# ALVI-Labs/frankenstein

Hardware: AMD Instinct MI355X
Metric: neural frames/sec (train fwd+bwd+AdamW, whole job) (higher is better)
Workload: dtype bf16; 1 GPU; brainformer-small (6L d=384 6x64 heads, N=6144 tokens) + 2-block perceiver, L1 head; fwd+bwd+clip+AdamW; per_gpu_batch=32, global_batch=32, frames_T=600, electrodes=256, parallelism=dp1, weights=random-init (seed 42)

## Files before the change

frankenstein_amd/_lib.py:

```python
from __future__ import annotations

import ctypes as C
from pathlib import Path

import os

LIB_PATH = Path(os.environ.get("FRANKEN_HIP_LIB") or Path(__file__).resolve().parent / "libfranken_hip.so")

FK_F32, FK_BF16 = 0, 1
MASK_NONE, MASK_CAUSAL, MASK_BLOCK_CAUSAL, MASK_PREFIX, MASK_KEYPAD, MASK_DENSE = 0, 1, 2, 3, 4, 5
NORM_LAYER, NORM_RMS = 0, 1
ATTN_Q_PRESCALED = 1
GEMV_GELU = 1
NT_RING2, NT_RING192, NT_RING128, NT_BIG, NT_GLDS4, NT_GLDS, NT_STAGED = range(7)
NT_ROUTE_F32 = -2

_p, _i64, _int, _f32, _f64, _sz, _u32 = C.c_void_p, C.c_int64, C.c_int, C.c_float, C.c_double, C.c_size_t, C.c_uint32

SIGNATURES = {
    "fk_version": (_int, []),
    "fk_last_error": (C.c_char_p, []),
    "fk_gemm_nt": (_int, [_p, _i64, _p, _i64, _p, _i64, _i64, _i64, _i64, _p, _p, _i64, _i64, _int, _int, _p]),
    "fk_gemv_nt": (_int, [_p, _i64, _p, _i64, _p, _i64, _i64, _i64, _i64, _p, _p, _i64, _p, _p, _f32, _int, _int, _int, _p]),
    "fk_gemm_nt_rope": (_int, [_p, _i64, _p, _i64, _p, _i64, _i64, _i64, _i64, _p, _p, _i64, _i64, _i64, _i64, _i64, _i64, _i64, _int, _p]),
    "fk_gemm_nt_swiglu": (_int, [_p, _i64, _p, _i64, _p, _i64, _p, _i64, _i64, _i64, _i64, _int, _p]),
    "fk_gemm_nt_dswiglu": (_int, [_p, _i64, _p, _i64, _p, _i64, _p, _i64, _i64, _i64, _i64, _int, _p]),
    "fk_mlp_bwd_fused": (_int, [_p, _i64, _p, _i64, _p, _i64, _p, _i64, _p, _i64, _p, _i64, _i64, _i64, _i64, _int, _p]),
    "fk_gemm_nt_route": (_int, [_i64, _i64, _i64, _int, _int, _int, _int]),
    "fk_gemm_tn_route": (_int, [_i64, _i64, _i64, _int, _p, _p]),
    "fk_gemm_tn_workspace_bytes": (_sz, [_i64, _i64, _i64, _int]),
    "fk_gemm_tn": (_int, [_p, _i64, _p, _i64, _p, _i64, _i64, _i64, _i64, _int, _int, _p, _sz, _p]),
    "fk_colsum_workspace_bytes": (_sz, [_i64, _i64]),
    "fk_colsum": (_int, [_p, _i64, _p, _i64, _i64, _int, _int, _p, _sz, _p]),
    "fk_attn_fwd": (_int, [_p, _p, _p, _p, _p] + [_i64] * 13 + [_int, _i64, _i64, _i64, _p, _p, _f32, _int, _int, _p]),
    "fk_attn_bwd": (_int, [_p] * 10 + [_i64] * 13 + [_int, _i64, _i64, _i64, _p, _p, _f32, _p, _i64, _i64, _int, _int, _p]),
    "fk_attn_fwd_dropout": (_int, [_p, _p, _p, _p, _p] + [_i64] * 13 + [_int, _i64, _i64, _i64, _p, _p, _f32, _int, _f32, _p, _u32, _int, _p]),
    "fk_attn_bwd_dropout": (_int, [_p] * 10 + [_i64] * 13 + [_int, _i64, _i64, _i64, _p, _p, _f32, _p, _i64, _i64, _int, _f32, _p, _u32, _int, _p]),
    "fk_dropout": (_int, [_p, _p, _p, _i64, _f32, _p, _u32, _int, _p]),
    "fk_norm_fwd": (_int, [_p, _p, _p, _p, _p, _p, _i64, _i64, _f32, _int, _int, _p]),
    "fk_norm_bwd_workspace_bytes": (_sz, [_i64, _i64]),
    "fk_norm_bwd": (_int, [_p] * 9 + [_i64, _i64, _int, _int, _int, _p, _sz, _p]),
    "fk_rope": (_int, [_p, _i64, _i64, _i64, _i64, _i64, _p, _i64, _i64, _int, _int, _p]),
    "fk_patchify": (_int, [_p, _p, _i64, _i64, _i64, _i64, _i64, _int, _p]),
    "fk_swiglu_fwd": (_int, [_p, _p, _i64, _i64, _int, _p]),
    "fk_swiglu_bwd": (_int, [_p, _p, _p, _i64, _i64, _int, _p]),
    "fk_gelu_fwd": (_int, [_p, _p, _i64, _int, _p]),
    "fk_gelu_bwd": (_int, [_p, _p, _p, _i64, _int, _p]),
    "fk_cast_pack": (_int, [_p, _i64, _p, _i64, _i64, _i64, _int, _int, _p]),
    "fk_cast_pack_rows": (_int, [_p, _i64, _p, _i64, _i64, _i64, _int, _i64, _i64, _i64, _int, _p]),
    "fk_cast_pack_multi": (_int, [_p, _i64, _i64, _int, _p]),
    "fk_cast": (_int, [_p, _int, _p, _int, _i64, _p]),
    "fk_add": (_int, [_p, _p, _p, _i64, _int, _p]),
    "fk_gather_rows": (_int, [_p, _i64, _int, _p, _i64, _p, _i64, _int, _i64, _i64, _i64, _int, _p]),
    "fk_scatter_add_rows": (_int, [_p, _int, _p, _i64, _p, _i64, _i64, _p]),
    "fk_prefix_mask": (_int, [_p, _p, _i64, _p, _p, _i64, _i64, _i64, _p]),
    "fk_copy2d": (_int, [_p, _i64, _p, _i64, _i64, _i64, _int, _p]),
    "fk_attn_combine": (_int, [_p, _p, _p, _p, _i64, _i64, _i64, _i64, _i64, _int, _p]),
    "fk_add2d": (_int, [_p, _i64, _p, _i64, _i64, _i64, _p]),
    "fk_gpt_embed_step": (_int, [_p, _p, _p, _p, _p, _i64, _i64, _i64, _int, _p]),
    "fk_kv_append": (_int, [_p, _p, _p, _i64, _i64, _i64, _int, _p]),
    "fk_attn_decode": (_int, [_p, _i64, _p, _i64, _i64, _p, _i64, _p, _i64, _i64, _i64, _f32, _int, _p]),
    "fk_sample_topk": (_int, [_p, _i64, _i64, _i64, _f32, _i64, _p, _p, _p, _p, _p, _i64, _i64, _p, _p]),
    "fk_attn_decode_beam": (_int, [_p, _i64, _p, _i64, _i64, _p, _i64, _p, _i64, _p, _i64, _i64, _i64, _f32, _int, _p]),
    "fk_beam_topk": (_int, [_p, _i64, _i64, _i64, _f32, _i64, _p, _p, _p]),
# ... 64 lines not shown
```

frankenstein_amd/csrc/gemm.hip:

```cpp
#include <type_traits>

#include "fk_common.h"

namespace {

#ifndef FK_EPI_UNROLL
#define FK_EPI_UNROLL 1
#endif
#include "gemm_tile.h"

struct NtArgs {
  const void* A; const void* B; void* C;
  const void* bias; const void* res;
  int64_t lda, ldb, ldc, ldr, res_rows;
  int M, N, K, vec_epi;
  int mode;
  void* aux; int64_t ldaux;
  const float* rope_table; int64_t rope_bs; int rope_T, rope_off, rope_D, rope_cols;
  int rope_qcols; int64_t rope_qoff;
};

#ifndef FK_NT_STORES_GEMM
#define FK_NT_STORES_GEMM 1
#endif
// ... 1054 lines not shown
#pragma unroll
      for (int i = 0; i < 2; ++i) tn_frag<T>(fa[i], as, wm * 64 + i * 32, s, lane);
#pragma unroll
      for (int j = 0; j < 2; ++j) tn_frag<T>(fb[j], bs, wn * 64 + j * 32, s, lane);
#pragma unroll
      for (int i = 0; i < 2; ++i)
#pragma unroll
        for (int j = 0; j < 2; ++j) mma32<T>(acc[i][j], fa[i], fb[j]);
    }
    if (kt + 1 < nk) lstore((kt + 1) & 1);
    __syncthreads();
  }

  float* out = (p.nsplit > 1) ? p.ws + (int64_t)split * p.N1 * p.N2 : p.C;
  const int64_t ldo = (p.nsplit > 1) ? p.N2 : p.ldc;
  const bool accum = (p.nsplit == 1) && p.accumulate;
#pragma unroll
  for (int j = 0; j < 2; ++j) {
    const int n = b0 + wn * 64 + j * 32 + li;
    if (n >= p.N2) continue;
#pragma unroll
    for (int i = 0; i < 2; ++i)
#pragma unroll
      for (int r = 0; r < 16; ++r) {
        const int m = a0 + wm * 64 + i * 32 + acc_row(r, lh);
        if (m >= p.N1) continue;
        float* dst = out + (int64_t)m * ldo + n;
        *dst = accum ? (*dst + acc[i][j][r]) : acc[i][j][r];
      }
  }
}

constexpr int TG_A = 384, TG_B = 128, TG_K = 32;
#ifndef FK_TG_NS
#define FK_TG_NS 4
#endif
constexpr int TG_NS = FK_TG_NS;
constexpr int TG_A_ROW = TG_A * 2, TG_B_ROW = TG_B * 2;
constexpr int TG_A_BYTES = TG_K * TG_A_ROW, TG_B_BYTES = TG_K * TG_B_ROW, TG_STAGE = TG_A_BYTES + TG_B_BYTES;

template <int PITCH> FK_DEV int tg_off(int row, int bytecol) {
  return row * PITCH + (bytecol & ~255) + ((((bytecol >> 6) ^ row) & 3) << 6) + (bytecol & 63);
}
template <int OFF> FK_DEV bf16x4 tr_read(unsigned base) {
  s16x4 r;
  asm volatile("ds_read_b64_tr_b16 %0, %1 offset:%2" : "=v"(r) : "v"(base), "n"(OFF) : "memory");
  return __builtin_bit_cast(bf16x4, r);
}
template <int N> FK_DEV void lgkm_wait() {
  asm volatile("s_waitcnt lgkmcnt(%0)" ::"n"(N) : "memory");
  __builtin_amdgcn_sched_barrier(0);
}
template <int PITCH, int S> FK_DEV void tg_frag(Frag<bf16_t>& f, unsigned base) {
  const bf16x4 v0 = tr_read<(16 * S) * PITCH>(base), v1 = tr_read<(16 * S + 4) * PITCH>(base);
#pragma unroll
  for (int e = 0; e < 4; ++e) { f.v[e] = v0[e]; f.v[4 + e] = v1[e]; }
}
FK_DEV unsigned lds_addr(const char* p) {
  return (unsigned)(__UINTPTR_TYPE__)((__attribute__((address_space(3))) const char*)p);
}

template <int TB>
__global__ __launch_bounds__(512, 2) void gemm_tn_big_kernel(TnArgs p) {
  constexpr int B_ROW = TB == 128 ? 256 : 512, B_BYTES = TG_K * B_ROW, STAGE = TG_A_BYTES + B_BYTES, NJ = TB / 64, WB = TB / 2;
  using T = bf16_t;
  extern __shared__ __attribute__((aligned(16))) char smem[];
  const int tid = threadIdx.x, lane = tid & 63;
  const int wave = __builtin_amdgcn_readfirstlane(tid >> 6);
  const int wm = wave >> 1, wn = wave & 1, li = lane & 31, lh = lane >> 5;
  const int nt2 = p.N2 / TB, ntiles = (p.N1 / TG_A) * nt2;
  const unsigned L = xcd_remap(blockIdx.x, gridDim.x);
  const int split = (int)(L / ntiles), tile = (int)(L % ntiles);
  const int a0 = (tile / nt2) * TG_A, b0 = (tile % nt2) * TB;
  const int mbeg = split * p.rows_per_split;
  const int mend = min(p.M, mbeg + p.rows_per_split);
  const int nk = (mend - mbeg) / TG_K;

  constexpr int APW = TG_A_BYTES / 8192, BPW = B_BYTES / 8192, PER = APW + BPW;
  const T* srcA[APW];
  const T* srcB[BPW];
#pragma unroll
  for (int j = 0; j < APW; ++j) {
    const int o = (wave * APW + j) * 1024 + lane * 16, row = o / TG_A_ROW, bc = o % TG_A_ROW;
    const int sc = (bc & ~255) + ((((bc >> 6) ^ row) & 3) << 6) + (bc & 63);
    srcA[j] = (const T*)p.A + (int64_t)(mbeg + row) * p.lda + a0 + sc / 2;
  }
#pragma unroll
  for (int j = 0; j < BPW; ++j) {
    const int o = (wave * BPW + j) * 1024 + lane * 16, row = o / B_ROW, bc = o % B_ROW;
    int sc = (bc & ~255) + ((((bc >> 6) ^ row) & 3) << 6) + (bc & 63);
    if (sc >= TB * 2) sc = 0;
    srcB[j] = (const T*)p.B + (int64_t)(mbeg + row) * p.ldb + b0 + sc / 2;
  }
  const int64_t astep = (int64_t)TG_K * p.lda, bstep = (int64_t)TG_K * p.ldb;
  auto stage = [&](int buf) {
    char* as = smem + buf * STAGE;
#pragma unroll
    for (int j = 0; j < APW; ++j) {
      __builtin_amdgcn_global_load_lds((glb_void_t*)srcA[j], (lds_void_t*)(as + (wave * APW + j) * 1024), 16, 0, 0);
      srcA[j] += astep;
    }
#pragma unroll
    for (int j = 0; j < BPW; ++j) {
      __builtin_amdgcn_global_load_lds((glb_void_t*)srcB[j], (lds_void_t*)(as + TG_A_BYTES + (wave * BPW + j) * 1024), 16, 0, 0);
      srcB[j] += bstep;
    }
  };

  unsigned fbase[3 + NJ];
  {
    const int g = lane >> 4, i = lane & 15, row = 8 * (g >> 1) + (i >> 2), dc = 16 * (g & 1) + 4 * (i & 3);
#pragma unroll
    for (int q = 0; q < 3; ++q) fbase[q] = lds_addr(smem) + tg_off<TG_A_ROW>(row, (wm * 96 + q * 32 + dc) * 2);
#pragma unroll
    for (int q = 0; q < NJ; ++q) fbase[3 + q] = lds_addr(smem) + TG_A_BYTES + tg_off<B_ROW>(row, (wn * WB + q * 32 + dc) * 2);
  }

  f32x16 acc[3][NJ];
#pragma unroll
  for (int i = 0; i < 3; ++i)
#pragma unroll
    for (int j = 0; j < NJ; ++j)
#pragma unroll
      for (int r = 0; r < 16; ++r) acc[i][j][r] = 0.0f;

#pragma unroll
  for (int s = 0; s < TG_NS - 1; ++s)
    if (s < nk) stage(s);
  int slot = 0;
  for (int kt = 0; kt < nk; ++kt) {
    const int after = nk - 1 - kt;
    if (after >= TG_NS - 2) vm_wait_barrier<(TG_NS - 2) * PER>();
    else if (after == 3) vm_wait_barrier<3 * PER>();
    else if (after == 2) vm_wait_barrier<2 * PER>();
    else if (after == 1) vm_wait_barrier<PER>();
    else vm_wait_barrier<0>();
    if (kt + TG_NS - 1 < nk) stage(slot == 0 ? TG_NS - 1 : slot - 1);
    const unsigned bo = slot * STAGE;
    slot = slot == TG_NS - 1 ? 0 : slot + 1;
    Frag<T> f0[3 + NJ], f1[3 + NJ];
#pragma unroll
    for (int q = 0; q < 3; ++q) tg_frag<TG_A_ROW, 0>(f0[q], fbase[q] + bo);
#pragma unroll
    for (int q = 0; q < NJ; ++q) tg_frag<B_ROW, 0>(f0[3 + q], fbase[3 + q] + bo);
#pragma unroll
    for (int q = 0; q < 3; ++q) tg_frag<TG_A_ROW, 1>(f1[q], fbase[q] + bo);
#pragma unroll
    for (int q = 0; q < NJ; ++q) tg_frag<B_ROW, 1>(f1[3 + q], fbase[3 + q] + bo);
    lgkm_wait<2 * (3 + NJ)>();
#pragma unroll
    for (int i = 0; i < 3; ++i)
#pragma unroll
      for (int j = 0; j < NJ; ++j) mma32<T>(acc[i][j], f0[i], f0[3 + j]);
    lgkm_wait<0>();
#pragma unroll
    for (int i = 0; i < 3; ++i)
#pragma unroll
      for (int j = 0; j < NJ; ++j) mma32<T>(acc[i][j], f1[i], f1[3 + j]);
  }

  float* out = (p.nsplit > 1) ? p.ws + (int64_t)split * p.N1 * p.N2 : p.C;
  const int64_t ldo = (p.nsplit > 1) ? p.N2 : p.ldc;
  const bool accum = (p.nsplit == 1) && p.accumulate;
#pragma unroll
  for (int j = 0; j < NJ; ++j) {
    const int n = b0 + wn * WB + j * 32 + li;
#pragma unroll
    for (int i = 0; i < 3; ++i)
#pragma unroll
      for (int r = 0; r < 16; ++r) {
        const int m = a0 + wm * 96 + i * 32 + acc_row(r, lh);
        float* dst = out + (int64_t)m * ldo + n;
        *dst = accum ? (*dst + acc[i][j][r]) : acc[i][j][r];
      }
  }
}

__global__ __launch_bounds__(256) void reduce_slabs4_kernel(const float* ws, float* C, int64_t ldc, int N1, int N2, int nsplit, int accumulate) {
  const int64_t total = (int64_t)N1 * N2, total4 = total >> 2;
  const int n2v = N2 >> 2;
  for (int64_t i = blockIdx.x * (int64_t)blockDim.x + threadIdx.x; i < total4; i += (int64_t)gridDim.x * blockDim.x) {
    const f32x4* src = reinterpret_cast<const f32x4*>(ws) + i;
    f32x4 s = {0.0f, 0.0f, 0.0f, 0.0f};
    int k = 0;
    for (; k + 8 <= nsplit; k += 8) {
      f32x4 v[8];
#pragma unroll
      for (int u = 0; u < 8; ++u) v[u] = src[(int64_t)(k + u) * total4];
#pragma unroll
      for (int u = 0; u < 8; ++u) s += v[u];
    }
    for (; k < nsplit; ++k) s += src[(int64_t)k * total4];
    f32x4* dst = reinterpret_cast<f32x4*>(C + (i / n2v) * ldc + (i % n2v) * 4);
    if (accumulate) s += *dst;
    *dst = s;
  }
}
__global__ void reduce_slabs_kernel(const float* ws, float* C, int64_t ldc, int N1, int N2, int nsplit, int accumulate) {
  const int64_t total = (int64_t)N1 * N2;
  for (int64_t i = blockIdx.x * (int64_t)blockDim.x + threadIdx.x; i < total; i += (int64_t)gridDim.x * blockDim.x) {
    float s = 0.0f;
    for (int k = 0; k < nsplit; ++k) s += ws[k * total + i];
    float* dst = C + (i / N2) * ldc + (i % N2);
    *dst = accumulate ? (*dst + s) : s;
  }
}

template <typename T>
__global__ __launch_bounds__(256) void colsum_partial_kernel(const T* X, int64_t ld, float* part, int rows, int cols, int rows_per_blk) {
  constexpr int N = 16 / sizeof(T);
  __shared__ float red[256 * N];
  const int r0 = blockIdx.y * rows_per_blk, r1 = min(rows, r0 + rows_per_blk);
  const int cvt = (cols + N - 1) / N;
  {
    const int cv0 = blockIdx.x * 256;
    const int cvn = min(256, cvt - cv0), groups = 256 / cvn;
    const int vec = threadIdx.x % cvn, grp = threadIdx.x / cvn;
    float acc[N];
#pragma unroll
    for (int e = 0; e < N; ++e) acc[e] = 0.0f;
    if (grp < groups) {
      const T* p = X + (int64_t)(cv0 + vec) * N;
      for (int r = r0 + grp; r < r1; r += groups) {
        if constexpr (sizeof(T) == 2) {
          bf16x8 v = *reinterpret_cast<const bf16x8*>(p + (int64_t)r * ld);
#pragma unroll
// ... 173 lines not shown
  FK_CHECK_ARG(lddh % 8 == 0 && ((uintptr_t)dH13 & 15) == 0, "fk_gemm_nt_dswiglu: dH13 must be 16-byte aligned with an 8-element stride");
  return launch_nt("fk_gemm_nt_dswiglu", dY, lda, W2T, ldb, dH13, lddh, M, H, K, nullptr, nullptr, 0, 0, dtype, dtype, 2,
                   const_cast<void*>(H13), ldh, stream);
}

int fk_gemm_nt_route(int64_t M, int64_t N, int64_t K, int dtype, int vec_epi, int mode, int has_rope) {
  FK_CHECK_ARG(dtype == FK_F32 || dtype == FK_BF16, "fk_gemm_nt_route: bad dtype %d", dtype);
  FK_CHECK_ARG(M > 0 && N > 0 && K > 0 && mode >= 0 && mode <= 2, "fk_gemm_nt_route: bad problem M=%lld N=%lld K=%lld mode=%d", (long long)M, (long long)N, (long long)K, mode);
  if (dtype == FK_F32) return FK_NT_ROUTE_F32;
  return (int)nt_route(M, N, K, dtype, vec_epi != 0, mode, has_rope != 0);
}

static int tn_plan(int64_t M, int64_t N1, int64_t N2, int dtype, int* nsplit, int64_t* rows_per_split) {
  const bool big = tn_big_ok(M, N1, N2, dtype);
  const int bkm = dtype == FK_BF16 ? 64 : 32;
  const int ns = big ? tn_big_splits(M, N1, N2) : tn_splits(M, N1, N2, bkm);
  if (nsplit) *nsplit = ns;
  if (rows_per_split) *rows_per_split = fk_cdiv(fk_cdiv(M, ns), bkm) * bkm;
  return big ? tn_big_tb(N1, N2) : 0;
}

int fk_gemm_tn_route(int64_t M, int64_t N1, int64_t N2, int dtype, int* nsplit, int64_t* rows_per_split) {
  FK_CHECK_ARG(dtype == FK_F32 || dtype == FK_BF16, "fk_gemm_tn_route: bad dtype %d", dtype);
  FK_CHECK_ARG(M > 0 && N1 > 0 && N2 > 0, "fk_gemm_tn_route: empty problem");
  return tn_plan(M, N1, N2, dtype, nsplit, rows_per_split);
}

size_t fk_gemm_tn_workspace_bytes(int64_t M, int64_t N1, int64_t N2, int dtype) {
  int ns;
  tn_plan(M, N1, N2, dtype, &ns, nullptr);
  return ns > 1 ? (size_t)ns * N1 * N2 * sizeof(float) : 0;
}

int fk_gemm_tn(const void* A, int64_t lda, const void* B, int64_t ldb, float* C, int64_t ldc, int64_t M, int64_t N1,
               int64_t N2, int accumulate, int dtype, void* workspace, size_t workspace_bytes, void* stream) {
  FK_CHECK_ARG(dtype == FK_F32 || dtype == FK_BF16, "fk_gemm_tn: bad dtype %d", dtype);
  const int vec = dtype == FK_BF16 ? 8 : 4;
  FK_CHECK_ARG(M > 0 && N1 > 0 && N2 > 0, "fk_gemm_tn: empty problem");
  FK_CHECK_ARG(M < (1LL << 31) && N1 < (1LL << 31) && N2 < (1LL << 31), "fk_gemm_tn: dims must fit int32");
  FK_CHECK_ARG(N1 % vec == 0 && N2 % vec == 0 && lda % vec == 0 && ldb % vec == 0,
               "fk_gemm_tn: N1/N2/lda/ldb must be multiples of %d (N1=%lld N2=%lld)", vec, (long long)N1, (long long)N2);
  FK_CHECK_ARG(((uintptr_t)A & 15) == 0 && ((uintptr_t)B & 15) == 0, "fk_gemm_tn: A/B must be 16-byte aligned");
  int ns;
  int64_t rps;
  const int tb = tn_plan(M, N1, N2, dtype, &ns, &rps);
  const bool big = tb != 0;
  const size_t need = ns > 1 ? (size_t)ns * N1 * N2 * sizeof(float) : 0;
  FK_CHECK_ARG(workspace_bytes >= need && (need == 0 || workspace), "fk_gemm_tn: workspace too small (%zu < %zu)", workspace_bytes, need);
  TnArgs p{A, B, C, (float*)workspace, lda, ldb, ldc, (int)M, (int)N1, (int)N2, (int)rps, ns, accumulate};
  dim3 grid((unsigned)(fk_cdiv(N1, BM) * fk_cdiv(N2, BN) * ns)), block(NTHREADS);
  hipStream_t s = (hipStream_t)stream;
  if (big) {
    dim3 bgrid((unsigned)((N1 / TG_A) * (N2 / tb) * ns));
    if (tb == 192) {
      constexpr int LDS192 = TG_NS * (TG_A_BYTES + TG_K * 512);
      fk_launch_lds<gemm_tn_big_kernel<192>>(bgrid, dim3(512), LDS192, s, p);
    } else {
      fk_launch_lds<gemm_tn_big_kernel<128>>(bgrid, dim3(512), TG_NS * TG_STAGE, s, p);
    }
  } else if (dtype == FK_BF16) hipLaunchKernelGGL((gemm_tn_kernel<bf16_t>), grid, block, 4 * TILE_BYTES, s, p);
  else hipLaunchKernelGGL((gemm_tn_kernel<float>), grid, block, 4 * TILE_BYTES, s, p);
  FK_CHECK_LAUNCH("fk_gemm_tn");
  if (ns > 1) {
    const int64_t total = N1 * N2;
    if (N2 % 4 == 0 && ldc % 4 == 0 && (((uintptr_t)C | (uintptr_t)workspace) & 15) == 0) {
      int nb = (int)fk_cdiv(total / 4, 256);
      if (nb > 2048) nb = 2048;
      hipLaunchKernelGGL(reduce_slabs4_kernel, dim3(nb), dim3(256), 0, s, (const float*)workspace, C, ldc, (int)N1, (int)N2, ns, accumulate);
    } else {
      int nb = (int)fk_cdiv(total, 256);
      if (nb > 2048) nb = 2048;
      hipLaunchKernelGGL(reduce_slabs_kernel, dim3(nb), dim3(256), 0, s, (const float*)workspace, C, ldc, (int)N1, (int)N2, ns, accumulate);
    }
    FK_CHECK_LAUNCH("fk_gemm_tn(reduce)");
  }
  return FK_OK;
}

size_t fk_colsum_workspace_bytes(int64_t rows, int64_t cols) { return (size_t)colsum_blocks(rows) * cols * sizeof(float); }

int fk_colsum(const void* X, int64_t ld, float* out, int64_t rows, int64_t cols, int accumulate, int dtype,
              void* workspace, size_t workspace_bytes, void* stream) {
  FK_CHECK_ARG(dtype == FK_F32 || dtype == FK_BF16, "fk_colsum: bad dtype %d", dtype);
  FK_CHECK_ARG(rows > 0 && cols > 0 && rows < (1LL << 31) && cols < (1LL << 31), "fk_colsum: bad shape");
  const int nb = colsum_blocks(rows);
  FK_CHECK_ARG(workspace && workspace_bytes >= (size_t)nb * cols * sizeof(float), "fk_colsum: workspace too small");
  const int rpb = (int)fk_cdiv(rows, nb);
  hipStream_t s = (hipStream_t)stream;
  const int vec = dtype == FK_BF16 ? 8 : 4;
  if (cols % vec == 0 && ld % vec == 0 && ((uintptr_t)X & 15) == 0) {
    dim3 grid((unsigned)fk_cdiv(fk_cdiv(cols, vec), 256), (unsigned)nb), block(256);
    if (dtype == FK_BF16) hipLaunchKernelGGL(colsum_partial_kernel<bf16_t>, grid, block, 0, s, (const bf16_t*)X, ld, (float*)workspace, (int)rows, (int)cols, rpb);
    else hipLaunchKernelGGL(colsum_partial_kernel<float>, grid, block, 0, s, (const float*)X, ld, (float*)workspace, (int)rows, (int)cols, rpb);
  } else {
    dim3 grid((unsigned)fk_cdiv(cols, 256), (unsigned)nb), block(256);
    if (dtype == FK_BF16) hipLaunchKernelGGL(colsum_partial_scalar_kernel<bf16_t>, grid, block, 0, s, (const bf16_t*)X, ld, (float*)workspace, (int)rows, (int)cols, rpb);
    else hipLaunchKernelGGL(colsum_partial_scalar_kernel<float>, grid, block, 0, s, (const float*)X, ld, (float*)workspace, (int)rows, (int)cols, rpb);
  }
  FK_CHECK_LAUNCH("fk_colsum(partial)");
  hipLaunchKernelGGL(colsum_final_kernel, dim3((unsigned)fk_cdiv(cols, 64)), dim3(256), 0, s, (const float*)workspace, out, (int)cols, nb, accumulate);
  FK_CHECK_LAUNCH("fk_colsum(final)");
  return FK_OK;
}

}
```

frankenstein_amd/engine.py:

```python
from __future__ import annotations

from typing import List, Optional, Sequence, Tuple

import math
import os
import weakref

import torch

from . import kernels as K
from .kernels import Mask, NO_MASK

Tensor = torch.Tensor

_COMPUTE_DTYPE = torch.bfloat16
_EPOCH = 0


def set_compute_dtype(dtype) -> None:
    global _COMPUTE_DTYPE
    if isinstance(dtype, str):
        dtype = {"bf16": torch.bfloat16, "bfloat16": torch.bfloat16, "fp32": torch.float32, "float32": torch.float32}[dtype]
    assert dtype in (torch.bfloat16, torch.float32)
    _COMPUTE_DTYPE = dtype
# ... 11 lines not shown
_WGRAD_STREAM = None


def enable_wgrad_stream(on: bool = True):
    global _WGRAD_STREAM
    _WGRAD_STREAM = torch.cuda.Stream() if on else None
    return _WGRAD_STREAM


def wgrad_stream():
    return _WGRAD_STREAM


def _arena_grad(p: Tensor):
    g = p.grad
    return g if (g is not None and getattr(p, "_fk_arena", False) and g.is_contiguous()) else None


def wgrad(a: Tensor, b: Tensor, params: Sequence[Tensor], swiglu_interleaved: bool = False):
    side = _WGRAD_STREAM
    grads = [_arena_grad(p) for p in params]
    if any(g is None for g in grads):
        dw = K.gemm_tn(a, b)
        if swiglu_interleaved:
            return list(_deinterleave_rows(dw, params[0].shape[0]))
        return _split_rows(dw, params)
    if side is not None:
        side.wait_stream(torch.cuda.current_stream())
        a.record_stream(side)
        b.record_stream(side)
    with torch.cuda.stream(side if side is not None else torch.cuda.current_stream()):
        Kd = b.shape[1]
        adjacent = all(grads[i + 1].data_ptr() == grads[i].data_ptr() + grads[i].numel() * 4 for i in range(len(grads) - 1))
        if swiglu_interleaved:
            dw = K.gemm_tn(a, b)
            H = params[0].shape[0]
            v = dw.view(H // 4, 8 * Kd)
            K.add2d_(grads[0].view(H // 4, 4 * Kd), v[:, :4 * Kd])
            K.add2d_(grads[1].view(H // 4, 4 * Kd), v[:, 4 * Kd:])
        elif adjacent:
            n = sum(p.shape[0] for p in params)
            out = torch.as_strided(grads[0], (n, Kd), (Kd, 1))
            K.gemm_tn(a, b, out=out, accumulate=True)
        else:
            dw = K.gemm_tn(a, b)
            for g, part in zip(grads, _split_rows(dw, params)):
                K.add2d_(g.view(part.shape), part)
    return [None] * len(params)


def norm_bwd(dh: Tensor, x2: Tensor, ln_w: Tensor, ln_b: Optional[Tensor], mean: Tensor, rstd: Tensor, dres: Optional[Tensor] = None,
             kind: int = K.NORM_LAYER):
    gw = _arena_grad(ln_w)
    gb = _arena_grad(ln_b) if ln_b is not None else None
    if gw is not None and (ln_b is None or gb is not None):
        dx, _, _ = K.norm_bwd(dh, x2, ln_w.detach(), mean, rstd, dres=dres, kind=kind, want_beta=ln_b is not None,
                              dgamma=gw.view(-1), dbeta=None if gb is None else gb.view(-1), accumulate=True)
        return dx, None, None
    return K.norm_bwd(dh, x2, ln_w.detach(), mean, rstd, dres=dres, kind=kind, want_beta=ln_b is not None)


class _Shadow:
    __slots__ = ("stamp", "tensor", "jobs", "params", "dtype", "ptrs", "repack")

    def __init__(self):
        self.stamp, self.tensor, self.jobs, self.params, self.dtype, self.ptrs = None, None, [], (), None, ()
        self.repack = None
# ... 878 lines not shown
```

frankenstein_amd/kernels.py:

```python
from __future__ import annotations

import math
from typing import Optional, Tuple

import torch

from . import _lib
from ._lib import FK_BF16, FK_F32, MASK_BLOCK_CAUSAL, MASK_CAUSAL, MASK_DENSE, MASK_KEYPAD, MASK_NONE, MASK_PREFIX, NORM_LAYER, NORM_RMS, ATTN_Q_PRESCALED, call, lib

Tensor = torch.Tensor


TIMERS = None
TIMER_PREFIX = None


class _timed:
    __slots__ = ("name", "ev")

    def __init__(self, name):
        self.name = name

    def __enter__(self):
        self.ev = None
# ... 161 lines not shown

def gemm_nt_route(M: int, N: int, K: int, dtype=torch.bfloat16, vec_epi: bool = True, mode: int = 0, has_rope: bool = False) -> int:
    r = lib().fk_gemm_nt_route(M, N, K, fk_dtype(dtype), int(vec_epi), mode, int(has_rope))
    if r == -1:
        _lib.check(r, "fk_gemm_nt_route")
    return r


def gemm_tn_route(M: int, N1: int, N2: int, dtype=torch.bfloat16) -> Tuple[int, int, int]:
    import ctypes
    ns, rps = ctypes.c_int(0), ctypes.c_int64(0)
    r = lib().fk_gemm_tn_route(M, N1, N2, fk_dtype(dtype), ctypes.byref(ns), ctypes.byref(rps))
    if r < 0:
        _lib.check(r, "fk_gemm_tn_route")
    return r, ns.value, rps.value


def gemm_tn(a: Tensor, b: Tensor, out: Optional[Tensor] = None, accumulate: bool = False) -> Tensor:
    assert a.dim() == 2 and b.dim() == 2 and a.shape[0] == b.shape[0] and a.dtype == b.dtype
    assert a.stride(1) == 1 and b.stride(1) == 1
    M, N1 = a.shape
    N2 = b.shape[1]
    if out is None:
        assert not accumulate
        out = torch.empty((N1, N2), dtype=torch.float32, device=a.device)
    assert out.shape == (N1, N2) and out.dtype == torch.float32 and out.stride(1) == 1
    ws, nb = _ws(lib().fk_gemm_tn_workspace_bytes(M, N1, N2, fk_dtype(a)), a.device)
    with _timed(f"gemm_tn:{M}x{N1}x{N2}"):
        call("fk_gemm_tn", a.data_ptr(), a.stride(0), b.data_ptr(), b.stride(0), out.data_ptr(), out.stride(0), M, N1, N2,
             int(accumulate), fk_dtype(a), _ptr(ws), nb, _stream())
    return out


def colsum(x: Tensor, out: Optional[Tensor] = None, accumulate: bool = False) -> Tensor:
    assert x.dim() == 2 and x.stride(1) == 1
    rows, cols = x.shape
    if out is None:
        assert not accumulate
        out = torch.empty(cols, dtype=torch.float32, device=x.device)
    assert out.numel() == cols and out.dtype == torch.float32 and out.is_contiguous()
    ws, nb = _ws(lib().fk_colsum_workspace_bytes(rows, cols), x.device)
    call("fk_colsum", x.data_ptr(), x.stride(0), out.data_ptr(), rows, cols, int(accumulate), fk_dtype(x), _ptr(ws), nb,
         _stream())
    return out


class Mask:
    __slots__ = ("kind", "c", "q_off", "k_off", "limits", "qfirst")

    def __init__(self, kind: int = MASK_NONE, c: int = 0, q_off: int = 0, k_off: int = 0, limits=None, qfirst=None):
        self.kind, self.c, self.q_off, self.k_off, self.limits, self.qfirst = kind, c, q_off, k_off, limits, qfirst

    def sliced(self, n_full_q: int, n_full_k: int, t_q: int, t_k: int) -> "Mask":
        assert self.kind not in (MASK_PREFIX, MASK_KEYPAD, MASK_DENSE) or (n_full_q == t_q and n_full_k == t_k), "table masks cannot be sliced"
        return Mask(self.kind, self.c, self.q_off + n_full_q - t_q, self.k_off + n_full_k - t_k, self.limits, self.qfirst)

    @staticmethod
    def from_dense(mask: Tensor, t_q: int, t_k: int) -> "Mask":
        assert mask.dim() >= 2
        m = mask[..., max(0, mask.shape[-2] - t_q):, max(0, mask.shape[-1] - t_k):]
        if m.dim() > 4:
            if any(d != 1 for d in m.shape[:-4]):
                raise NotImplementedError(f"dense attention mask {tuple(mask.shape)}: at most [B, H, N_q, N_k]")
            m = m.reshape(m.shape[-4:])
        while m.dim() < 4:
            m = m.unsqueeze(0)
# ... 671 lines not shown
```

include/franken_hip.h:

```cpp
#ifndef FRANKEN_HIP_H
#define FRANKEN_HIP_H

#include <stddef.h>
#include <stdint.h>

#ifdef __cplusplus
extern "C" {
#endif

#define FK_VERSION 302

#define FK_OK 0
#define FK_EINVAL (-1)
#define FK_ELAUNCH (-2)
#define FK_EUNSUPPORTED (-3)

enum { FK_F32 = 0, FK_BF16 = 1 };
enum { FK_MASK_NONE = 0, FK_MASK_CAUSAL = 1, FK_MASK_BLOCK_CAUSAL = 2, FK_MASK_PREFIX = 3, FK_MASK_KEYPAD = 4, FK_MASK_DENSE = 5 };
enum { FK_ATTN_Q_PRESCALED = 1 };
enum { FK_NORM_LAYER = 0, FK_NORM_RMS = 1 };
enum { FK_ACT_SWIGLU = 0, FK_ACT_GELU = 1 };
enum { FK_GEMV_GELU = 1 };

int fk_version(void);
const char* fk_last_error(void);

int fk_gemm_nt(const void* A, int64_t lda, const void* B, int64_t ldb, void* C, int64_t ldc, int64_t M, int64_t N,
               int64_t K, const void* bias, const void* residual, int64_t ldr, int64_t res_rows, int dtype,
               int out_dtype, void* stream);
int fk_gemv_nt(const void* A, int64_t lda, const void* W, int64_t ldw, void* C, int64_t ldc, int64_t M, int64_t N, int64_t K,
               const void* bias, const void* residual, int64_t ldr, const float* ln_gamma, const float* ln_beta, float ln_eps,
               int flags, int dtype, int out_dtype, void* stream);
int fk_gemm_nt_rope(const void* A, int64_t lda, const void* B, int64_t ldb, void* C, int64_t ldc, int64_t M, int64_t N,
                    int64_t K, const void* bias, const float* table, int64_t table_bs, int64_t T, int64_t pos_off, int64_t D,
                    int64_t rot_cols, int64_t q_cols, int64_t q_table_off, int dtype, void* stream);
int fk_gemm_nt_swiglu(const void* A, int64_t lda, const void* W13, int64_t ldb, void* H13, int64_t ldh, void* G,
                      int64_t ldg, int64_t M, int64_t H, int64_t K, int dtype, void* stream);
int fk_gemm_nt_dswiglu(const void* dY, int64_t lda, const void* W2T, int64_t ldb, const void* H13, int64_t ldh, void* dH13,
                       int64_t lddh, int64_t M, int64_t H, int64_t K, int dtype, void* stream);
int fk_mlp_bwd_fused(const void* dY, int64_t lddy, const void* W2T, int64_t ldw2t, const void* H13, int64_t ldh, const void* W13T,
                     int64_t ldw13t, void* dH13, int64_t lddh, void* dX, int64_t lddx, int64_t M, int64_t H, int64_t D, int dtype,
                     void* stream);
enum { FK_NT_RING2 = 0, FK_NT_RING192 = 1, FK_NT_RING128 = 2, FK_NT_BIG = 3, FK_NT_GLDS4 = 4, FK_NT_GLDS = 5, FK_NT_STAGED = 6 };
#define FK_NT_ROUTE_F32 (-2)
int fk_gemm_nt_route(int64_t M, int64_t N, int64_t K, int dtype, int vec_epi, int mode, int has_rope);
size_t fk_gemm_tn_workspace_bytes(int64_t M, int64_t N1, int64_t N2, int dtype);
int fk_gemm_tn(const void* A, int64_t lda, const void* B, int64_t ldb, float* C, int64_t ldc, int64_t M, int64_t N1,
               int64_t N2, int accumulate, int dtype, void* workspace, size_t workspace_bytes, void* stream);
int fk_gemm_tn_route(int64_t M, int64_t N1, int64_t N2, int dtype, int* nsplit, int64_t* rows_per_split);
size_t fk_colsum_workspace_bytes(int64_t rows, int64_t cols);
int fk_colsum(const void* X, int64_t ld, float* out, int64_t rows, int64_t cols, int accumulate, int dtype,
              void* workspace, size_t workspace_bytes, void* stream);

int fk_attn_fwd(const void* Q, const void* K, const void* V, void* O, float* LSE, int64_t B, int64_t H, int64_t Nq,
                int64_t Nk, int64_t D, int64_t q_bs, int64_t q_rs, int64_t k_bs, int64_t k_rs, int64_t v_bs,
                int64_t v_rs, int64_t o_bs, int64_t o_rs, int mask_kind, int64_t mask_c, int64_t q_off, int64_t k_off,
                const int32_t* limits, const int32_t* qfirst, float scale, int flags, int dtype, void* stream);
int fk_attn_bwd(const void* Q, const void* K, const void* V, const void* O, const void* dO, const float* LSE,
                void* dQ, void* dK, void* dV, float* delta_ws, int64_t B, int64_t H, int64_t Nq, int64_t Nk, int64_t D,
                int64_t q_bs, int64_t q_rs, int64_t k_bs, int64_t k_rs, int64_t v_bs, int64_t v_rs, int64_t o_bs,
                int64_t o_rs, int mask_kind, int64_t mask_c, int64_t q_off, int64_t k_off, const int32_t* limits,
                const int32_t* qfirst, float scale, const float* rope_table, int64_t rope_bs, int64_t rope_off, int flags,
                int dtype, void* stream);

int fk_attn_fwd_dropout(const void* Q, const void* K, const void* V, void* O, float* LSE, int64_t B, int64_t H, int64_t Nq,
                        int64_t Nk, int64_t D, int64_t q_bs, int64_t q_rs, int64_t k_bs, int64_t k_rs, int64_t v_bs,
                        int64_t v_rs, int64_t o_bs, int64_t o_rs, int mask_kind, int64_t mask_c, int64_t q_off, int64_t k_off,
                        const int32_t* limits, const int32_t* qfirst, float scale, int flags, float drop_p, const uint32_t* drop_seed,
                        uint32_t drop_site, int dtype, void* stream);
int fk_attn_bwd_dropout(const void* Q, const void* K, const void* V, const void* O, const void* dO, const float* LSE,
                        void* dQ, void* dK, void* dV, float* delta_ws, int64_t B, int64_t H, int64_t Nq, int64_t Nk, int64_t D,
                        int64_t q_bs, int64_t q_rs, int64_t k_bs, int64_t k_rs, int64_t v_bs, int64_t v_rs, int64_t o_bs,
                        int64_t o_rs, int mask_kind, int64_t mask_c, int64_t q_off, int64_t k_off, const int32_t* limits,
                        const int32_t* qfirst, float scale, const float* rope_table, int64_t rope_bs, int64_t rope_off, int flags,
                        float drop_p, const uint32_t* drop_seed, uint32_t drop_site, int dtype, void* stream);

int fk_dropout(const void* x, const void* res, void* y, int64_t n, float p, const uint32_t* seed, uint32_t site, int dtype, void* stream);

int fk_norm_fwd(const void* x, const float* gamma, const float* beta, void* y, float* mean, float* rstd,
                int64_t rows, int64_t dim, float eps, int kind, int dtype, void* stream);
size_t fk_norm_bwd_workspace_bytes(int64_t rows, int64_t dim);
// ... 132 lines not shown
```

Measured before the change: 404,100 frames/s.

## Software-pipeline TN GEMM fragment loads and fuse SwiGLU weight-grad de-interleave into reduce

Restructures the TN weight-gradient GEMM main loop so LDS fragment reads for the next k-step and the global-to-LDS DMA pieces are interleaved between individual MFMA instructions, replacing the per-iteration stage/load/compute sequence. It also adds a swiglu variant whose split-K reduce kernel writes interleaved up/gate rows straight into the two separate fp32 gradient buffers with accumulation. This drops the temporary dw tensor and the host-side view/add de-interleave in the engine. The cost is more register pressure from double-buffered fragments, tighter scheduling constraints, and the swiglu path only applies when a split plan exists.

```diff
diff --git a/frankenstein_amd/_lib.py b/frankenstein_amd/_lib.py
--- a/frankenstein_amd/_lib.py
+++ b/frankenstein_amd/_lib.py
@@ -30,6 +30,7 @@
     "fk_gemm_tn_route": (_int, [_i64, _i64, _i64, _int, _p, _p]),
     "fk_gemm_tn_workspace_bytes": (_sz, [_i64, _i64, _i64, _int]),
     "fk_gemm_tn": (_int, [_p, _i64, _p, _i64, _p, _i64, _i64, _i64, _i64, _int, _int, _p, _sz, _p]),
+    "fk_gemm_tn_swiglu": (_int, [_p, _i64, _p, _i64, _p, _p, _i64, _i64, _i64, _i64, _int, _p, _sz, _p]),
     "fk_colsum_workspace_bytes": (_sz, [_i64, _i64]),
     "fk_colsum": (_int, [_p, _i64, _p, _i64, _i64, _int, _int, _p, _sz, _p]),
     "fk_attn_fwd": (_int, [_p, _p, _p, _p, _p] + [_i64] * 13 + [_int, _i64, _i64, _i64, _p, _p, _f32, _int, _int, _p]),
diff --git a/frankenstein_amd/csrc/gemm.hip b/frankenstein_amd/csrc/gemm.hip
--- a/frankenstein_amd/csrc/gemm.hip
+++ b/frankenstein_amd/csrc/gemm.hip
@@ -1110,10 +1110,7 @@
 }
 
 constexpr int TG_A = 384, TG_B = 128, TG_K = 32;
-#ifndef FK_TG_NS
-#define FK_TG_NS 4
-#endif
-constexpr int TG_NS = FK_TG_NS;
+constexpr int TG_NS = 4;
 constexpr int TG_A_ROW = TG_A * 2, TG_B_ROW = TG_B * 2;
 constexpr int TG_A_BYTES = TG_K * TG_A_ROW, TG_B_BYTES = TG_K * TG_B_ROW, TG_STAGE = TG_A_BYTES + TG_B_BYTES;
 
@@ -1171,17 +1168,14 @@
     srcB[j] = (const T*)p.B + (int64_t)(mbeg + row) * p.ldb + b0 + sc / 2;
   }
   const int64_t astep = (int64_t)TG_K * p.lda, bstep = (int64_t)TG_K * p.ldb;
-  auto stage = [&](int buf) {
+  auto piece = [&](int buf, int j) __attribute__((always_inline)) {
     char* as = smem + buf * STAGE;
-#pragma unroll
-    for (int j = 0; j < APW; ++j) {
+    if (j < APW) {
       __builtin_amdgcn_global_load_lds((glb_void_t*)srcA[j], (lds_void_t*)(as + (wave * APW + j) * 1024), 16, 0, 0);
       srcA[j] += astep;
-    }
-#pragma unroll
-    for (int j = 0; j < BPW; ++j) {
-      __builtin_amdgcn_global_load_lds((glb_void_t*)srcB[j], (lds_void_t*)(as + TG_A_BYTES + (wave * BPW + j) * 1024), 16, 0, 0);
-      srcB[j] += bstep;
+    } else {
+      __builtin_amdgcn_global_load_lds((glb_void_t*)srcB[j - APW], (lds_void_t*)(as + TG_A_BYTES + (wave * BPW + j - APW) * 1024), 16, 0, 0);
+      srcB[j - APW] += bstep;
     }
   };
 
@@ -1202,39 +1196,75 @@
 #pragma unroll
       for (int r = 0; r < 16; ++r) acc[i][j][r] = 0.0f;
 
+  static_assert(TG_NS == 4, "the waits below count one stage in flight behind the awaited one");
+  constexpr int NF = 3 + NJ, NM = 3 * NJ;
+  constexpr int RPG = 2, DMA0 = NM - 1 - PER;
+  Frag<T> f0[NF], f1[NF];
+  auto frag = [&](Frag<T>* f, auto S, int q, unsigned bo) __attribute__((always_inline)) {
+    if (q < 3) tg_frag<TG_A_ROW, decltype(S)::value>(f[q], fbase[q] + bo);
+    else tg_frag<B_ROW, decltype(S)::value>(f[q], fbase[q] + bo);
+  };
+  auto mma = [&](Frag<T>* f, int m) __attribute__((always_inline)) {
+#ifndef FK_TN_PROBE_NOMMA
+    mma32<T>(acc[m / NJ][m % NJ], f[m / NJ], f[3 + m % NJ]);
+#endif
+  };
+  using S0 = std::integral_constant<int, 0>;
+  using S1 = std::integral_constant<int, 1>;
+  int slot = 0;
+  auto step = [&](auto NEXT, auto DMA, auto VM) __attribute__((always_inline)) {
+    const unsigned bo = slot * STAGE;
+    const int prev = slot == 0 ? TG_NS - 1 : slot - 1;
+    slot = slot == TG_NS - 1 ? 0 : slot + 1;
+    const unsigned nbo = slot * STAGE;
+#ifndef FK_TN_PROBE_HOIST
+#pragma unroll
+    for (int q = 0; q < NF; ++q) frag(f1, S1{}, q, bo);
+#endif
+    lgkm_wait<2 * NF>();
+#pragma unroll
+    for (int m = 0; m < NM; ++m) mma(f0, m);
+    __builtin_amdgcn_sched_barrier(0);
+    if constexpr (decltype(NEXT)::value) vm_wait_barrier<decltype(VM)::value>();
+    lgkm_wait<0>();
+#pragma unroll
+    for (int m = 0; m < NM; ++m) {
+      mma(f1, m);
+      __builtin_amdgcn_sched_barrier(0);
+#ifndef FK_TN_PROBE_HOIST
+      if constexpr (decltype(NEXT)::value)
+#pragma unroll
+        for (int q = RPG * m; q < RPG * (m + 1); ++q)
+          if (q < NF) frag(f0, S0{}, q, nbo);
+#endif
+#ifndef FK_TN_PROBE_NODMA
+      if constexpr (decltype(DMA)::value) if (m >= DMA0 && m < DMA0 + PER) piece(prev, m - DMA0);
+#endif
+      __builtin_amdgcn_sched_barrier(0);
+    }
+  };
+  using Yes = std::true_type;
+  using No = std::false_type;
+  using Vm0 = std::integral_constant<int, 0>;
+  using Vm1 = std::integral_constant<int, PER>;
 #pragma unroll
   for (int s = 0; s < TG_NS - 1; ++s)
-    if (s < nk) stage(s);
-  int slot = 0;
-  for (int kt = 0; kt < nk; ++kt) {
-    const int after = nk - 1 - kt;
-    if (after >= TG_NS - 2) vm_wait_barrier<(TG_NS - 2) * PER>();
-    else if (after == 3) vm_wait_barrier<3 * PER>();
-    else if (after == 2) vm_wait_barrier<2 * PER>();
-    else if (after == 1) vm_wait_barrier<PER>();
-    else vm_wait_barrier<0>();
-    if (kt + TG_NS - 1 < nk) stage(slot == 0 ? TG_NS - 1 : slot - 1);
-    const unsigned bo = slot * STAGE;
-    slot = slot == TG_NS - 1 ? 0 : slot + 1;
-    Frag<T> f0[3 + NJ], f1[3 + NJ];
-#pragma unroll
-    for (int q = 0; q < 3; ++q) tg_frag<TG_A_ROW, 0>(f0[q], fbase[q] + bo);
-#pragma unroll
-    for (int q = 0; q < NJ; ++q) tg_frag<B_ROW, 0>(f0[3 + q], fbase[3 + q] + bo);
-#pragma unroll
-    for (int q = 0; q < 3; ++q) tg_frag<TG_A_ROW, 1>(f1[q], fbase[q] + bo);
-#pragma unroll
-    for (int q = 0; q < NJ; ++q) tg_frag<B_ROW, 1>(f1[3 + q], fbase[3 + q] + bo);
-    lgkm_wait<2 * (3 + NJ)>();
-#pragma unroll
-    for (int i = 0; i < 3; ++i)
-#pragma unroll
-      for (int j = 0; j < NJ; ++j) mma32<T>(acc[i][j], f0[i], f0[3 + j]);
-    lgkm_wait<0>();
-#pragma unroll
-    for (int i = 0; i < 3; ++i)
-#pragma unroll
-      for (int j = 0; j < NJ; ++j) mma32<T>(acc[i][j], f1[i], f1[3 + j]);
+    if (s < nk)
+#pragma unroll
+      for (int j = 0; j < PER; ++j) piece(s, j);
+  if (nk > 0) {
+    if (nk >= 3) vm_wait_barrier<2 * PER>(); else if (nk == 2) vm_wait_barrier<PER>(); else vm_wait_barrier<0>();
+#pragma unroll
+    for (int q = 0; q < NF; ++q) frag(f0, S0{}, q, 0);
+#ifdef FK_TN_PROBE_HOIST
+#pragma unroll
+    for (int q = 0; q < NF; ++q) frag(f1, S1{}, q, 0);
+#endif
+    int kt = 0;
+    for (; kt + TG_NS - 1 < nk; ++kt) step(Yes{}, Yes{}, Vm1{});
+    if (kt + 2 < nk) { step(Yes{}, No{}, Vm1{}); ++kt; }
+    if (kt + 1 < nk) step(Yes{}, No{}, Vm0{});
+    step(No{}, No{}, Vm0{});
   }
 
   float* out = (p.nsplit > 1) ? p.ws + (int64_t)split * p.N1 * p.N2 : p.C;
@@ -1254,7 +1284,8 @@
   }
 }
 
-__global__ __launch_bounds__(256) void reduce_slabs4_kernel(const float* ws, float* C, int64_t ldc, int N1, int N2, int nsplit, int accumulate) {
+template <bool IL>
+__global__ __launch_bounds__(256) void reduce_slabs4_kernel(const float* ws, float* C, float* C1, int64_t ldc, int N1, int N2, int nsplit, int accumulate) {
   const int64_t total = (int64_t)N1 * N2, total4 = total >> 2;
   const int n2v = N2 >> 2;
   for (int64_t i = blockIdx.x * (int64_t)blockDim.x + threadIdx.x; i < total4; i += (int64_t)gridDim.x * blockDim.x) {
@@ -1269,7 +1300,13 @@
       for (int u = 0; u < 8; ++u) s += v[u];
     }
     for (; k < nsplit; ++k) s += src[(int64_t)k * total4];
-    f32x4* dst = reinterpret_cast<f32x4*>(C + (i / n2v) * ldc + (i % n2v) * 4);
+    int64_t r = i / n2v;
+    float* base = C;
+    if constexpr (IL) {
+      if (r & 4) base = C1;
+      r = (r >> 3) * 4 + (r & 3);
+    }
+    f32x4* dst = reinterpret_cast<f32x4*>(base + r * ldc + (i % n2v) * 4);
     if (accumulate) s += *dst;
     *dst = s;
   }
@@ -1509,8 +1546,8 @@
   return ns > 1 ? (size_t)ns * N1 * N2 * sizeof(float) : 0;
 }
 
-int fk_gemm_tn(const void* A, int64_t lda, const void* B, int64_t ldb, float* C, int64_t ldc, int64_t M, int64_t N1,
-               int64_t N2, int accumulate, int dtype, void* workspace, size_t workspace_bytes, void* stream) {
+static int launch_tn(const void* A, int64_t lda, const void* B, int64_t ldb, float* C, float* C1, int64_t ldc, int64_t M, int64_t N1,
+                     int64_t N2, int accumulate, int dtype, void* workspace, size_t workspace_bytes, void* stream) {
   FK_CHECK_ARG(dtype == FK_F32 || dtype == FK_BF16, "fk_gemm_tn: bad dtype %d", dtype);
   const int vec = dtype == FK_BF16 ? 8 : 4;
   FK_CHECK_ARG(M > 0 && N1 > 0 && N2 > 0, "fk_gemm_tn: empty problem");
@@ -1524,6 +1561,9 @@
   const bool big = tb != 0;
   const size_t need = ns > 1 ? (size_t)ns * N1 * N2 * sizeof(float) : 0;
   FK_CHECK_ARG(workspace_bytes >= need && (need == 0 || workspace), "fk_gemm_tn: workspace too small (%zu < %zu)", workspace_bytes, need);
+  if (C1)
+    FK_CHECK_ARG(ns > 1 && N1 % 8 == 0 && N2 % 4 == 0 && ldc % 4 == 0 && (((uintptr_t)C | (uintptr_t)C1 | (uintptr_t)workspace) & 15) == 0,
+                 "fk_gemm_tn_swiglu: needs a split plan (see fk_gemm_tn_route), N1 %% 8 == 0, N2 %% 4 == 0 and 16-byte aligned destinations");
   TnArgs p{A, B, C, (float*)workspace, lda, ldb, ldc, (int)M, (int)N1, (int)N2, (int)rps, ns, accumulate};
   dim3 grid((unsigned)(fk_cdiv(N1, BM) * fk_cdiv(N2, BN) * ns)), block(NTHREADS);
   hipStream_t s = (hipStream_t)stream;
@@ -1543,7 +1583,8 @@
     if (N2 % 4 == 0 && ldc % 4 == 0 && (((uintptr_t)C | (uintptr_t)workspace) & 15) == 0) {
       int nb = (int)fk_cdiv(total / 4, 256);
       if (nb > 2048) nb = 2048;
-      hipLaunchKernelGGL(reduce_slabs4_kernel, dim3(nb), dim3(256), 0, s, (const float*)workspace, C, ldc, (int)N1, (int)N2, ns, accumulate);
+      if (C1) hipLaunchKernelGGL(reduce_slabs4_kernel<true>, dim3(nb), dim3(256), 0, s, (const float*)workspace, C, C1, ldc, (int)N1, (int)N2, ns, accumulate);
+      else hipLaunchKernelGGL(reduce_slabs4_kernel<false>, dim3(nb), dim3(256), 0, s, (const float*)workspace, C, C1, ldc, (int)N1, (int)N2, ns, accumulate);
     } else {
       int nb = (int)fk_cdiv(total, 256);
       if (nb > 2048) nb = 2048;
@@ -1552,6 +1593,17 @@
     FK_CHECK_LAUNCH("fk_gemm_tn(reduce)");
   }
   return FK_OK;
+}
+
+int fk_gemm_tn(const void* A, int64_t lda, const void* B, int64_t ldb, float* C, int64_t ldc, int64_t M, int64_t N1,
+               int64_t N2, int accumulate, int dtype, void* workspace, size_t workspace_bytes, void* stream) {
+  return launch_tn(A, lda, B, ldb, C, nullptr, ldc, M, N1, N2, accumulate, dtype, workspace, workspace_bytes, stream);
+}
+
+int fk_gemm_tn_swiglu(const void* A, int64_t lda, const void* B, int64_t ldb, float* d_up, float* d_gate, int64_t ldc, int64_t M,
+                      int64_t H, int64_t N2, int dtype, void* workspace, size_t workspace_bytes, void* stream) {
+  FK_CHECK_ARG(d_up && d_gate && H > 0 && H % 4 == 0, "fk_gemm_tn_swiglu: needs both destinations and H %% 4 == 0");
+  return launch_tn(A, lda, B, ldb, d_up, d_gate, ldc, M, 2 * H, N2, 1, dtype, workspace, workspace_bytes, stream);
 }
 
 size_t fk_colsum_workspace_bytes(int64_t rows, int64_t cols) { return (size_t)colsum_blocks(rows) * cols * sizeof(float); }
diff --git a/frankenstein_amd/engine.py b/frankenstein_amd/engine.py
--- a/frankenstein_amd/engine.py
+++ b/frankenstein_amd/engine.py
@@ -67,7 +67,9 @@
     with torch.cuda.stream(side if side is not None else torch.cuda.current_stream()):
         Kd = b.shape[1]
         adjacent = all(grads[i + 1].data_ptr() == grads[i].data_ptr() + grads[i].numel() * 4 for i in range(len(grads) - 1))
-        if swiglu_interleaved:
+        if swiglu_interleaved and K.gemm_tn_swiglu_ok(a, b, grads[0], grads[1]):
+            K.gemm_tn_swiglu_(a, b, grads[0], grads[1])
+        elif swiglu_interleaved:
             dw = K.gemm_tn(a, b)
             H = params[0].shape[0]
             v = dw.view(H // 4, 8 * Kd)
diff --git a/frankenstein_amd/kernels.py b/frankenstein_amd/kernels.py
--- a/frankenstein_amd/kernels.py
+++ b/frankenstein_amd/kernels.py
@@ -217,6 +217,26 @@
     return out
 
 
+def gemm_tn_swiglu_ok(a: Tensor, b: Tensor, d_up: Tensor, d_gate: Tensor) -> bool:
+    M, N1 = a.shape
+    N2 = b.shape[1]
+    return (gemm_tn_route(M, N1, N2, a.dtype)[1] > 1 and N1 % 8 == 0 and N2 % 4 == 0 and d_up.is_contiguous() and d_gate.is_contiguous()
+            and d_up.data_ptr() % 16 == 0 and d_gate.data_ptr() % 16 == 0)
+
+
+def gemm_tn_swiglu_(a: Tensor, b: Tensor, d_up: Tensor, d_gate: Tensor) -> None:
+    assert a.dim() == 2 and b.dim() == 2 and a.shape[0] == b.shape[0] and a.dtype == b.dtype
+    assert a.stride(1) == 1 and b.stride(1) == 1
+    M, N1 = a.shape
+    N2 = b.shape[1]
+    for d in (d_up, d_gate):
+        assert d.shape == (N1 // 2, N2) and d.dtype == torch.float32 and d.is_contiguous()
+    ws, nb = _ws(lib().fk_gemm_tn_workspace_bytes(M, N1, N2, fk_dtype(a)), a.device)
+    with _timed(f"gemm_tn_swiglu:{M}x{N1}x{N2}"):
+        call("fk_gemm_tn_swiglu", a.data_ptr(), a.stride(0), b.data_ptr(), b.stride(0), d_up.data_ptr(), d_gate.data_ptr(), N2, M, N1 // 2,
+             N2, fk_dtype(a), _ptr(ws), nb, _stream())
+
+
 def colsum(x: Tensor, out: Optional[Tensor] = None, accumulate: bool = False) -> Tensor:
     assert x.dim() == 2 and x.stride(1) == 1
     rows, cols = x.shape
diff --git a/include/franken_hip.h b/include/franken_hip.h
--- a/include/franken_hip.h
+++ b/include/franken_hip.h
@@ -47,6 +47,8 @@
 size_t fk_gemm_tn_workspace_bytes(int64_t M, int64_t N1, int64_t N2, int dtype);
 int fk_gemm_tn(const void* A, int64_t lda, const void* B, int64_t ldb, float* C, int64_t ldc, int64_t M, int64_t N1,
                int64_t N2, int accumulate, int dtype, void* workspace, size_t workspace_bytes, void* stream);
+int fk_gemm_tn_swiglu(const void* A, int64_t lda, const void* B, int64_t ldb, float* d_up, float* d_gate, int64_t ldc, int64_t M,
+                      int64_t H, int64_t N2, int dtype, void* workspace, size_t workspace_bytes, void* stream);
 int fk_gemm_tn_route(int64_t M, int64_t N1, int64_t N2, int dtype, int* nsplit, int64_t* rows_per_split);
 size_t fk_colsum_workspace_bytes(int64_t rows, int64_t cols);
 int fk_colsum(const void* X, int64_t ld, float* out, int64_t rows, int64_t cols, int accumulate, int dtype,
```

New measurement: 408,200 frames/s (median of 6 runs). +1.0%, better.
